# Shamir-Lab/Faucet

Hardware: AMD Instinct MI355X
Metric: canonical k-mers/s (load+scan) at k=31, 100bp reads; % HBM roofline (higher is better)
Workload: dtype u64

## Files before the change

### faucet_amd/_lib.py

```python
from __future__ import annotations

import ctypes as C
import os

HERE = os.path.dirname(os.path.abspath(__file__))
LIB_PATH = os.path.join(HERE, "libfaucet_gpu.so")

OK, ERR_ARG, ERR_HIP, ERR_STATE, ERR_CAPACITY, ERR_NOMEM = range(6)
BLOO1, BLOO2 = 0, 1
FLAG_PROFILE = 1
FLAG_EAGER_FLAGS = 2
FLAG_NO_RESIDENT = 4
FLAG_RECORD_STOPS = 8
FLAG_MERCY = 16
FLAG_KEY_ORDER_FROM_START = 32
STOP_POS_MASK, STOP_FORWARD, STOP_FIRST, STOP_FAKE = 0x0FFFFFFF, 1 << 28, 1 << 29, 1 << 30
TABLE_ENTRY_BYTES = 32


class Params(C.Structure):
    _fields_ = [("k", C.c_int32), ("j", C.c_int32), ("max_spacer_dist", C.c_int32), ("n_hash", C.c_int32),
                ("tai", C.c_uint64), ("device", C.c_int32), ("flags", C.c_int32), ("junction_capacity", C.c_uint64),
                ("max_batch_bases", C.c_uint64), ("stream", C.c_void_p), ("walk_window_span", C.c_uint64)]

# ... 105 lines not shown
    "fgpu_probe_bloom_junction": (C.c_int, [_vp, _vp, _u64, _vp]),
    "fgpu_stage3_set_junctions": (C.c_int, [_vp, _vp, _vp, _u64]),
    "fgpu_stage3_find_neighbors": (C.c_int, [_vp, _vp, _vp, _u64, _i32, _vp, _P(_u64), _vp, _u64]),
    "fgpu_stage3_contig_words": (_u64, [_i32, _i32]),
    "fgpu_kernel_times": (C.c_int, [_vp, _P(KernelTime), C.c_int]),
    "fgpu_kernel_times_reset": (C.c_int, [_vp]),
    "fgpu_profile_enable": (C.c_int, [_vp, C.c_int]),
    "fgpu_diag_stream_copy": (C.c_int, [_vp, _u64, C.c_int, _P(_f64)]),
    "fgpu_diag_random_access": (C.c_int, [_vp, _u64, _u64, C.c_int, C.c_int, _P(_f64)]),
    "fgpu_diag_ko_trace": (C.c_int, [_vp, _vp, _u64, _P(_u64)]),
    "fgpu_diag_ko_stamps": (C.c_int, [_vp, _vp, _u64, _P(_u64)]),
    "fgpu_diag_binned_chain": (C.c_int, [_vp, _u64, _u64, _u64, C.c_int, C.c_int, C.c_int, _P(_f64), _P(_f64), _P(_f64), _P(_f64), _P(_f64), _P(C.c_int)]),
    "fgpu_diag_device_attr": (C.c_int, [_vp, _P(_i32), _P(_i32), _P(_i32), _P(_i32)]),
    "fgpu_diag_walk_probe": (C.c_int, [_vp, _P(_u64)]),
    "fgpu_diag_load_split": (C.c_int, [_vp, _P(_u64), _P(_u64)]),
    "fgpu_diag_scan_replays": (C.c_int, [_vp, _P(_u64)]),
    "fgpu_diag_host_waits": (C.c_int, [_vp, _P(_u64), _P(_f64)]),
    "fgpu_diag_load_tables": (C.c_int, [_vp, _u64, _P(_f64), _P(_f64), _P(_f64)]),
    "fgpu_diag_pair_placements": (C.c_int, [_vp, C.c_int, _u64, _P(_f64)]),
    "fgpu_diag_late_flags": (C.c_int, [_vp, _P(_u64)]),
    "fgpu_diag_binned_probes": (C.c_int, [_vp, _u64, _u64, _u64, C.c_int, _P(_f64), _P(_f64), _P(_f64), _P(_f64)]),
    "fgpu_scan_pairs_devptr": (C.c_int, [_vp, C.c_int, _P(_vp), _P(_u64)]),
    "fgpu_device_alloc": (C.c_int, [_vp, _u64, _P(_vp)]),
    "fgpu_device_free": (C.c_int, [_vp, _vp]),
    "fgpu_device_copy": (C.c_int, [_vp, _vp, _vp, _u64]),
    "fgpu_device_zero": (C.c_int, [_vp, _vp, _u64]),
    "fgpu_group_create": (C.c_int, [C.c_int, C.c_int, _P(_vp)]),
    "fgpu_group_destroy": (None, [_vp]),
    "fgpu_group_attach": (C.c_int, [_vp, C.c_int, _vp]),
    "fgpu_group_abort": (None, [_vp]),
# ... 39 lines not shown
```

### faucet_amd/api.py

```python
from __future__ import annotations

import ctypes as C

import numpy as np

from . import _lib as L


class FaucetGpuError(RuntimeError):
    pass


def _check(rc, ctx=None):
    if rc != L.OK:
        msg = L.load().fgpu_last_error(ctx).decode(errors="replace") if ctx is not None else L.load().fgpu_last_error(None).decode()
        raise FaucetGpuError(f"libfaucet_gpu error {rc}: {msg}")


def solve_p1(estimated_kmers: int, singletons: int, fp: float = 0.04) -> float:
    it = C.c_int32(0)
    p1 = L.load().fgpu_solve_p1(estimated_kmers, singletons, C.c_float(fp), C.byref(it))
    if p1 < 0:
        raise ValueError("p1 solver: root not bracketed (singletons must be > 0 and < estimated_kmers)")
    return p1
# ... 458 lines not shown
    def diag_scan_replays(self) -> int:
        n = C.c_uint64(0)
        self._c(self.lib.fgpu_diag_scan_replays(self.h, C.byref(n)))
        return int(n.value)

    def diag_late_flags(self) -> dict:
        out = (C.c_uint64 * 3)()
        self._c(self.lib.fgpu_diag_late_flags(self.h, out))
        return {"noted": int(out[0]), "conflicts": int(out[1]), "swept": int(out[2])}

    def diag_load_split(self) -> dict:
        a, b = C.c_uint64(0), C.c_uint64(0)
        self._c(self.lib.fgpu_diag_load_split(self.h, C.byref(a), C.byref(b)))
        return {"in_mark": int(a.value), "pending": int(b.value)}

    def diag_binned_probes(self, table_bytes: int, n_probes: int, slice_bytes: int = 4 << 20, iters: int = 3) -> dict:
        v = [C.c_double(0) for _ in range(4)]
        self._c(self.lib.fgpu_diag_binned_probes(self.h, table_bytes, n_probes, slice_bytes, iters, *[C.byref(x) for x in v]))
        return dict(zip(("direct_per_s", "binned_per_s", "bin_ms", "probe_ms"), [float(x.value) for x in v]))

    def diag_binned_chain(self, table_bytes: int, n_items: int, slice_bytes: int = 4 << 20, n_hash: int = 3, fill_byte: int = 0x29, iters: int = 3) -> dict:
        v = [C.c_double(0) for _ in range(5)]
        eq = C.c_int(0)
        self._c(self.lib.fgpu_diag_binned_chain(self.h, table_bytes, n_items, slice_bytes, n_hash, fill_byte, iters, *[C.byref(x) for x in v], C.byref(eq)))
        d = dict(zip(("direct_ms", "bin_ms", "first_ms", "rest_ms", "survivors_share"), [float(x.value) for x in v]))
        d["equal"] = bool(eq.value)
        return d

    def diag_ko_trace(self) -> np.ndarray:
        out = np.zeros((1 << 21, 4), dtype=np.uint64)
# ... 116 lines not shown
```

### faucet_amd/csrc/api.hip

```cpp
#include <cstdio>
#include <algorithm>
#include <string>

#include <chrono>
#include <thread>

#include "fgpu_ctx.h"

int fgpu_scan_export_impl(fgpu_ctx* ctx, void* dev_entries, uint64_t cap_entries, uint64_t* d_stamps, uint64_t* n_entries);
int fgpu_scan_import_impl(fgpu_ctx* ctx, const void* dev_entries, uint64_t n);
int fgpu_scan_download_impl(fgpu_ctx* ctx, uint64_t* keys_host, fgpu_junction* recs_host, uint64_t cap, uint64_t* n_out);

static thread_local std::string g_create_error;

int g_fgpu_trace = getenv("FGPU_TRACE") && getenv("FGPU_TRACE")[0] == '1';

int fgpu_ensure(fgpu_ctx* ctx, DevBuf* b, uint64_t bytes) {
    if (b->bytes >= bytes && b->p) return FGPU_OK;
    if (b->p) {
        FGPU_HIP(fgpu_sync_stream(ctx, ctx->stream));
        FGPU_HIP(hipFree(b->p));
        b->p = nullptr;
        b->bytes = 0;
    } else {
// ... 134 lines not shown
static bool is_pow2(uint64_t x) { return x && !(x & (x - 1)); }

static void journal_recycle(fgpu_ctx* ctx);
static int journal_add(fgpu_ctx* ctx, BatchBufs* b, const fgpu_reads* reads);
static int scan_replay(fgpu_ctx* ctx);

int fgpu_check_reads(fgpu_ctx* ctx, const fgpu_reads* r) {
    if (!r || (r->n_reads && (!r->bases || !r->offsets))) { ctx->err = "null read batch"; return FGPU_ERR_ARG; }
    return FGPU_OK;
}

void fgpu_load_pass_policy(fgpu_ctx* ctx) {
    static const char* carry_env = getenv("FGPU_CARRY_MODE");
    ctx->carry_by_set = carry_env ? carry_env[0] == 's' && carry_env[1] == 'e' : ctx->prm.tai == (1ULL << 31);
    ctx->epoch_positions = ctx->swept_positions = 0;
    ctx->sweep_num = ctx->sweep_den = 1;
    const char* sweep_env = getenv("FGPU_SWEEP_RATIO");
    if (sweep_env) {
        unsigned n = 1, d = 1;
        if (sscanf(sweep_env, "%u/%u", &n, &d) == 2 && d > 0) { ctx->sweep_num = n; ctx->sweep_den = d; }
    }
    {
        const char* e = getenv("FGPU_SWEEP_MIN_FRAC");
        const double frac = e ? atof(e) : 16.0;
        ctx->sweep_min = frac > 0.0 ? (uint64_t)((double)ctx->prm.tai / frac / (double)std::max(1, ctx->prm.n_hash)) : 0;
    }
}
int fgpu_load_pass_counters(fgpu_ctx* ctx) {
    FGPU_HIP(hipMemsetAsync(ctx->counters, 0, sizeof(DevCounters), ctx->stream));
    memset(&ctx->load_stats, 0, sizeof(ctx->load_stats));
// ... 193 lines not shown
    void* ptrs[] = {ctx->lp.bits, ctx->lp.first, ctx->short_pf, ctx->bloo1, ctx->bloo2, ctx->first, ctx->pair, ctx->rec, ctx->slice_first, ctx->slice_pair, ctx->jkeys, ctx->jrecs, ctx->jstamps, ctx->jfilter, ctx->wkeys,
                    ctx->wbits, ctx->uf_parent, ctx->cl_count, ctx->cl_offset, ctx->cl_fill, ctx->cl_fail, ctx->ko_hk, ctx->ko_occ, ctx->ko_piece, ctx->cl_members, ctx->cl_roots, ctx->counters,
                    ctx->wdesc};
    for (void* p : ptrs) if (p) hipFree(p);
    stop_queue_recycle(ctx);
    for (StopBatch& f : ctx->stop_pool) hipHostFree(f.data);
    ctx->stop_pool.clear();
    if (ctx->counters_host) hipHostFree(ctx->counters_host);
    if (ctx->fb_host) hipHostFree(ctx->fb_host);
    if (ctx->wstream) { hipStreamSynchronize(ctx->wstream); hipStreamDestroy(ctx->wstream); }
    if (ctx->cstream) { hipStreamSynchronize(ctx->cstream); hipStreamDestroy(ctx->cstream); }
    if (ctx->ostream) { hipStreamSynchronize(ctx->ostream); hipStreamDestroy(ctx->ostream); }
    if (ctx->ev_walked) hipEventDestroy(ctx->ev_walked);
    if (ctx->ev_listed) hipEventDestroy(ctx->ev_listed);
    if (ctx->ev_settled) hipEventDestroy(ctx->ev_settled);
    for (int q = 0; q < 2; q++) if (ctx->ev_uf_reset[q]) hipEventDestroy(ctx->ev_uf_reset[q]);
    if (ctx->own_stream && ctx->stream) hipStreamDestroy(ctx->stream);
    for (ResidentBatch* r : ctx->resident) delete r;
    for (PackedBlock* b : ctx->packed) delete b;
    for (JournalBatch* j : ctx->journal) delete j;
    for (JournalBatch* j : ctx->journal_pool) delete j;
    for (BatchBufs* b : ctx->all_batches) {
        if (b->pure_done) hipEventDestroy(b->pure_done);
        if (b->walk_done) hipEventDestroy(b->walk_done);
        delete b;
    }
    delete ctx;
}

int fgpu_synchronize(fgpu_ctx* ctx) {
// ... 29 lines not shown
        if (e != hipSuccess) {
            ctx->err = std::string("hipMalloc of the interleaved filter pair failed: ") + hipGetErrorString(e);
            ctx->pair = nullptr;
            return FGPU_ERR_NOMEM;
        }
        if (int rc = fgpu_place_pair(ctx)) return rc;
    }
    ctx->shard_times = (keep_carry & FGPU_LOAD_SHARD_TIMES) != 0;
    ctx->shard_planes = (keep_carry & FGPU_LOAD_SHARD_PLANES) != 0 && !ctx->shard_times && ctx->prm.n_hash <= 4;
    ctx->fixup_ready = false;
    ctx->scan_resident_base = 0;
    ctx->pass_positions = ctx->pass_batches = 0;
    ctx->pass_empty_carry = !(keep_carry & FGPU_LOAD_KEEP_CARRY);
    keep_carry &= FGPU_LOAD_KEEP_CARRY;
    fgpu_load_pass_policy(ctx);
    if (!ctx->rec_layout) FGPU_HIP(hipMemsetAsync(ctx->first, 0xFF, ctx->prm.tai * 4, ctx->stream));
    fgpu_resident_reset(ctx, true);
    if (!keep_carry) FGPU_HIP(hipMemsetAsync(ctx->bloo1, 0, ctx->bloom_bytes, ctx->stream));
    FGPU_HIP(hipMemsetAsync(ctx->bloo2, 0, ctx->bloom_bytes, ctx->stream));
    int rc = fgpu_load_pair_begin(ctx);
    if (rc) return rc;
    if ((rc = fgpu_load_pass_counters(ctx))) return rc;
    ctx->phase = 1;
    return FGPU_OK;
}

int fgpu_load_batch(fgpu_ctx* ctx, const fgpu_reads* reads) {
    if (!ctx) return FGPU_ERR_ARG;
    if (ctx->phase != 1) { ctx->err = "load_batch outside load_begin/load_end"; return FGPU_ERR_STATE; }
    int rc = fgpu_check_reads(ctx, reads);
// ... 875 lines not shown
    FGPU_HIP(hipMemcpy(&cnt, (const char*)ctx->ko_trace.p + 8, 8, hipMemcpyDeviceToHost));
    if (cnt > 4096) cnt = 4096;
    if (cnt * 1024 > cap_words) cnt = cap_words / 1024;
    if (cnt && out) FGPU_HIP(hipMemcpy(out, (const char*)ctx->ko_trace.p + (8ULL << 23), cnt * 1024 * 8, hipMemcpyDeviceToHost));
    *n_pieces = cnt;
    return FGPU_OK;
}

int fgpu_diag_load_split(fgpu_ctx* ctx, uint64_t* in_mark, uint64_t* pending) {
    if (!ctx || !in_mark || !pending) return FGPU_ERR_ARG;
    *in_mark = ctx->load_mark_hits;
    *pending = ctx->load_mark_pending;
    return FGPU_OK;
}

int fgpu_diag_ovw(fgpu_ctx* ctx, uint64_t out[6]) {
    if (!ctx || !out) return FGPU_ERR_ARG;
    for (int i = 0; i < 4; i++) out[i] = ctx->counters_host->ovw[i];
    out[4] = ctx->counters_host->ovw_kept;
    out[5] = ctx->counters_host->ko_overflows;
    return FGPU_OK;
}

int fgpu_diag_prepared_refresh(fgpu_ctx* ctx, uint64_t out[4]) {
    if (!ctx || !out) return FGPU_ERR_ARG;
    out[0] = ctx->refresh_full;
    out[1] = ctx->refresh_delta;
    out[2] = ctx->delta_keys;
    out[3] = ctx->refresh_mismatch;
    return FGPU_OK;
// ... 46 lines not shown
```

### faucet_amd/csrc/fgpu_ctx.h

```cpp
#pragma once
#include <chrono>
#include <hip/hip_runtime.h>
#include <stdint.h>
#include <stdio.h>
#include <string.h>

#include <string>
#include <thread>
#include <vector>

#include "../../include/faucet_gpu.h"
#include <deque>

#include "fgpu_device.h"

#define FGPU_PADW 8
#define FGPU_USUAL_SPAN (1ULL << 26)
#define FGPU_MAX_SPAN (1ULL << 26)

struct DevBuf {
    void*    p = nullptr;
    uint64_t bytes = 0;
};

struct BatchBufs {
    DevBuf codes, bad;
    DevBuf readflag;
    DevBuf pending;
    DevBuf sure;
    DevBuf fail;
    DevBuf same;
    DevBuf valid, pm, ps, ff, fb, cf0, cf1, cb0, cb1, inF, inB;
    DevBuf lk;
    DevBuf cand;
    uint32_t cand_gen = 0;
    DevBuf nF, nB, need;
    DevBuf kh;
    DevBuf cr;
    DevBuf ps_prefix;
    DevBuf pieces;
    DevBuf sF, sB;
    DevBuf piece_read;
    DevBuf stop_off, stop_out;
    const uint64_t* d_offs = nullptr;
    uint64_t seq = 0;
    bool stops_pending = false;
// ... 141 lines not shown
    int bg_rc = 0;
    std::string bg_err;

    uint32_t* bloo1 = nullptr;
    uint64_t epoch_positions = 0;
    uint64_t swept_positions = 0;
    bool shard_times = false;
    bool shard_planes = false;
    bool fixup_ready = false;
    uint64_t pass_positions = 0;
    uint32_t cur_tb = 0;
    bool pass_empty_carry = true;
    uint64_t pass_batches = 0;
    uint64_t sweep_min = 0;
    uint32_t sweep_num = 1, sweep_den = 1;
    bool carry_by_set = false;
    uint32_t* bloo2 = nullptr;
    uint32_t* first = nullptr;
    uint2* pair = nullptr;
    uint32_t* rec = nullptr;
    bool rec_layout = false;
    uint64_t bloom_bytes = 0;
    int phase = 0;
    uint64_t slice_lo = 0, slice_n = 0;
    uint32_t* slice_first = nullptr;
    uint2* slice_pair = nullptr;
    uint64_t slice_first_bytes = 0, slice_pair_bytes = 0;
    bool slice_committed = false;
    bool slice_mercy = false;
    bool slice_probe_owed = false;
// ... 283 lines not shown
```

### faucet_amd/csrc/load.hip

```cpp
#include <algorithm>

#include "fgpu_ctx.h"
#include "fgpu_flags.h"
#include "load_common.h"

namespace {

template <int REC>
__global__ void __launch_bounds__(256) k_load_mark(const uint64_t* __restrict__ codes, const uint64_t* __restrict__ bad,
                                                   uint64_t T, uint64_t n_words, FdParams fp, Filt<REC> f, uint32_t tb,
                                                   uint64_t* __restrict__ pending, uint64_t plane_stride, uint64_t* __restrict__ sure, DevCounters* cnt) {
    unsigned long long n_ok = 0, n_hit = 0, n_pend = 0;
    const uint64_t total = n_words * 64;
    for (uint64_t p = (uint64_t)blockIdx.x * blockDim.x + threadIdx.x; p < total; p += (uint64_t)gridDim.x * blockDim.x) {
        bool ok = p < T && fd_window_ok(bad, p, fp.k);
        bool pend = false, hit = false;
        uint32_t miss_bits = 0;
        if (ok) {
            n_ok++;
            uint64_t canon = fd_canon(fd_kmer_at(codes, p, fp.k), fp.k);
            uint64_t hA, hB;
            fd_hash_pair(canon, fp.tai_mask, hA, hB);
            uint32_t missing = 0, b2_missing = 0;
            uint64_t h = hA;
// ... 263 lines not shown
        const int g = fd_lane() & 15;
        uint32_t lo = g < 8 ? nib << (4 * g) : 0u, hi = g >= 8 ? nib << (4 * (g - 8)) : 0u;
#pragma unroll
        for (int o = 1; o < 16; o <<= 1) {
            lo |= __shfl_xor(lo, o, 64);
            hi |= __shfl_xor(hi, o, 64);
        }
        if (g == 0) {
            const uint64_t w = i >> 3;
            if (lo) pair[w].x |= lo;
            if (hi) pair[w + 1].x |= hi;
        }
    }
}

template <int REC>
__global__ void __launch_bounds__(256) k_carry_set(const uint64_t* __restrict__ codes, const uint64_t* __restrict__ bad, uint64_t T,
                                                   uint64_t n_words, FdParams fp, Filt<REC> f, const uint64_t* __restrict__ sure) {
    const uint64_t total = n_words * 64;
    for (uint64_t p = (uint64_t)blockIdx.x * blockDim.x + threadIdx.x; p < total; p += (uint64_t)gridDim.x * blockDim.x) {
        if (!(p < T && fd_window_ok(bad, p, fp.k)) || ((sure[p >> 6] >> (p & 63)) & 1ULL)) continue;
        uint64_t hA, hB;
        fd_hash_pair(fd_canon(fd_kmer_at(codes, p, fp.k), fp.k), fp.tai_mask, hA, hB);
        uint64_t h = hA;
        for (int i = 0; i < fp.n_hash; i++) {
            const uint32_t bit = 1u << (h & 31);
            if (!(f.word(h)[0] & bit)) atomicOr(f.word(h), bit);
            h = (h + hB) & fp.tai_mask;
        }
    }
// ... 160 lines not shown
        ctx->resident_open = false;
        return FGPU_OK;
    }
    r->T = bb.T;
    r->n_words = bb.n_words;
    r->tb = ctx->cur_tb;
    FGPU_HIP(hipMemcpyAsync(r->codes.p, bb.codes.p, parts[0], hipMemcpyDeviceToDevice, ctx->stream));
    FGPU_HIP(hipMemcpyAsync(r->bad.p, bb.bad.p, pb, hipMemcpyDeviceToDevice, ctx->stream));
    FGPU_HIP(hipMemcpyAsync(r->sure.p, bb.sure.p, pb, hipMemcpyDeviceToDevice, ctx->stream));
    if (parts[3]) FGPU_HIP(hipMemcpyAsync(r->fail.p, bb.fail.p, parts[3], hipMemcpyDeviceToDevice, ctx->stream));
    ctx->resident_count++;
    ctx->resident_bytes += kept;
    return FGPU_OK;
}

int fgpu_load_sweep(fgpu_ctx* ctx) {
    if (ctx->epoch_positions == 0) return FGPU_OK;
    if (ctx->phase == 3) {
        if (ctx->slice_n) FGPU_LAUNCH("slice_carry_update", k_carry_from_first, 4096, 256, ctx->slice_pair, (const uint4*)ctx->slice_first, ctx->slice_n);
    } else if (ctx->rec_layout) {
        FGPU_LAUNCH("carry_update", k_carry_from_rec, 8192, 256, ctx->rec, ctx->prm.tai / 32);
    } else {
        FGPU_LAUNCH("carry_update", k_carry_from_first, 4096, 256, ctx->pair, (const uint4*)ctx->first, ctx->prm.tai);
    }
    ctx->swept_positions += ctx->epoch_positions;
    ctx->epoch_positions = 0;
    return FGPU_OK;
}

int fgpu_epoch_before_batch(fgpu_ctx* ctx, uint64_t span) {
    if (!ctx->carry_by_set && !ctx->shard_times && ctx->epoch_positions + span >= 0xFFFFFFF0ULL) return fgpu_load_sweep(ctx);
    return FGPU_OK;
}
int fgpu_epoch_after_batch(fgpu_ctx* ctx, uint64_t span) {
    if (ctx->carry_by_set) return FGPU_OK;
    ctx->epoch_positions += span;
    if (ctx->epoch_positions * ctx->sweep_den >= ctx->swept_positions * ctx->sweep_num && ctx->epoch_positions >= ctx->sweep_min) return fgpu_load_sweep(ctx);
    return FGPU_OK;
}

template <int REC>
static int load_batch(fgpu_ctx* ctx, const Filt<REC>& f, uint32_t tb, bool keep_fail) {
    BatchBufs& bb = *ctx->cur;
    const uint64_t plane_stride = bb.n_words + FGPU_PADW;
    const unsigned grid = fgpu_grid(bb.n_words * 64, 256);
    static const int resolve_sm = getenv("FGPU_RESOLVE_SM") ? atoi(getenv("FGPU_RESOLVE_SM")) : 4096;
    FGPU_LAUNCH("load_mark", k_load_mark<REC>, grid, 256, (const uint64_t*)bb.codes.p, (const uint64_t*)bb.bad.p, bb.T, bb.n_words, ctx->fd, f,
                tb, (uint64_t*)bb.pending.p, plane_stride, (uint64_t*)bb.sure.p, ctx->counters);
    if (ctx->fd.n_hash <= MISS_PLANES && resolve_sm && !keep_fail) {
        const unsigned rgrid = (unsigned)std::min<uint64_t>((bb.n_words + 255) / 256, (uint64_t)std::max(resolve_sm, 64));
        FGPU_LAUNCH("load_resolve", k_load_resolve_sm<REC>, rgrid, 256, (const uint64_t*)bb.codes.p, bb.n_words, ctx->fd, f, tb,
                    (const uint64_t*)bb.pending.p, plane_stride, (unsigned long long*)bb.sure.p, ctx->counters);
// ... 19 lines not shown

int fgpu_stage_load(fgpu_ctx* ctx) {
    BatchBufs& bb = *ctx->cur;
    if (bb.T == 0) return FGPU_OK;
    const uint64_t plane_stride = bb.n_words + FGPU_PADW;
    int rc = fgpu_ensure_b(ctx, &bb.pending, (MISS_PLANES + 1) * plane_stride * 8);
    if (rc) return rc;
    if ((rc = fgpu_ensure_b(ctx, &bb.sure, (bb.n_words + FGPU_PADW) * 8))) return rc;
    if ((rc = fgpu_util_count_segments(ctx, bb.bad.p, bb.n_words, ctx->fd.k))) return rc;
    const uint64_t span = bb.n_words * 64;
    if ((rc = fgpu_epoch_before_batch(ctx, span))) return rc;
    if (ctx->shard_times && ctx->pass_positions + span >= 0xFFFFFFF0ULL) {
        ctx->err = "FGPU_LOAD_SHARD_TIMES: the pass exceeds 2^32 stream positions (FGPU_LOAD_SHARD_PLANES has no such limit)";
        return FGPU_ERR_CAPACITY;
    }
    const uint32_t tb = ctx->shard_times ? (uint32_t)ctx->pass_positions : ctx->carry_by_set ? 0u : (uint32_t)ctx->epoch_positions;
    const bool keep_fail = ctx->shard_planes && ctx->fd.n_hash <= MISS_PLANES;
    if (keep_fail && (rc = fgpu_ensure_b(ctx, &bb.fail, MISS_PLANES * plane_stride * 8))) return rc;
    ctx->cur_tb = tb;
    ctx->pass_positions += span;
    if ((rc = with_layout(ctx, [&](auto f) { return load_batch(ctx, f, tb, keep_fail); }))) return rc;
    if ((rc = fgpu_epoch_after_batch(ctx, span))) return rc;
    return fgpu_resident_keep(ctx);
}

int fgpu_load_pair_begin(fgpu_ctx* ctx) {
    if (ctx->rec_layout) FGPU_LAUNCH("pair_join", k_rec_init, 8192, 256, ctx->rec, (const uint32_t*)ctx->bloo1, ctx->bloom_bytes / 4);
    else FGPU_LAUNCH("pair_join", k_pair_join, 2048, 256, ctx->pair, (const uint32_t*)ctx->bloo1, (const uint32_t*)nullptr, ctx->bloom_bytes / 4);
    return FGPU_OK;
}
int fgpu_load_pair_end(fgpu_ctx* ctx) {
    if (ctx->phase == 3) {
        FGPU_HIP(hipMemsetAsync(ctx->bloo1, 0, ctx->bloom_bytes, ctx->stream));
        FGPU_HIP(hipMemsetAsync(ctx->bloo2, 0, ctx->bloom_bytes, ctx->stream));
        if (ctx->slice_n)
            FGPU_LAUNCH("pair_split", k_pair_split, 2048, 256, (const uint2*)ctx->slice_pair, ctx->bloo1 + ctx->slice_lo / 32,
                        ctx->bloo2 + ctx->slice_lo / 32, ctx->slice_n / 32);
    } else if (ctx->rec_layout) {
        FGPU_LAUNCH("pair_split", k_rec_split, 4096, 256, (const uint32_t*)ctx->rec, ctx->bloo1, ctx->bloo2, ctx->bloom_bytes / 4);
    } else {
        FGPU_LAUNCH("pair_split", k_pair_split, 2048, 256, (const uint2*)ctx->pair, ctx->bloo1, ctx->bloo2, ctx->bloom_bytes / 4);
    }
    return FGPU_OK;
}

int fgpu_stage_fixup(fgpu_ctx* ctx, const uint32_t* prefix) {
// ... 55 lines not shown
```

### faucet_amd/csrc/scan_pure.hip

```cpp
#include <algorithm>

#include "fgpu_ctx.h"
#include "fgpu_flags.h"

namespace {

__global__ void __launch_bounds__(256) k_scan_same(const uint64_t* __restrict__ codes, const uint64_t* __restrict__ kept_codes, uint64_t n_code_words,
                                                   const uint64_t* __restrict__ bad, const uint64_t* __restrict__ kept_bad, uint64_t n_words,
                                                   uint32_t* same) {
    bool differ = false;
    for (uint64_t i = (uint64_t)blockIdx.x * blockDim.x + threadIdx.x; i < n_code_words; i += (uint64_t)gridDim.x * blockDim.x) {
        differ |= codes[i] != kept_codes[i];
        if (i < n_words) differ |= bad[i] != kept_bad[i];
    }
    if (__ballot(differ) && fd_lane() == 0) *same = 0;
}

__global__ void __launch_bounds__(256) k_scan_valid(const uint64_t* __restrict__ codes, const uint64_t* __restrict__ bad,
                                                    uint64_t T, uint64_t n_words, FdParams fp, const uint32_t* __restrict__ bloom,
                                                    const uint64_t* __restrict__ sure, const uint32_t* __restrict__ same,
                                                    uint64_t* __restrict__ valid, DevCounters* cnt) {
    unsigned long long n_ok = 0, n_reused = 0;
    const uint64_t total = n_words * 64;
    const bool reuse = sure && *same != 0;
// ... 419 lines not shown
        for (int nt = 0; nt < 4; nt++) {
            const uint64_t e = ((km << 2) | (uint64_t)nt) & fp.kmask;
            if (fd_bloom_contains_canon(bloom, fd_canon(e, fp.k), fp.tai_mask, fp.n_hash) && jcheck_dfs(e, fp, bloom)) {
                if (r != -1) { r = -2; break; }
                r = nt;
            }
        }
    } else {
        int paths = 0;
        for (int nt = 0; nt < 4; nt++) paths += jcheck_dfs(((km << 2) | (uint64_t)nt) & fp.kmask, fp, bloom) ? 1 : 0;
        r = paths > 1 ? 1 : 0;
    }
    out[i] = (signed char)r;
}

}

void fgpu_touch_scan_pure() {
    hipFuncAttributes attr;
    (void)hipFuncGetAttributes(&attr, (const void*)k_scan_same);
}

int fgpu_util_probe_stage3(fgpu_ctx* ctx, const uint64_t* d_kmers, uint64_t n, int mode, signed char* d_out) {
    FGPU_LAUNCH("probe_stage3", k_probe_stage3, fgpu_blocks(n, 256), 256, d_kmers, n, mode, ctx->fd, (const uint32_t*)ctx->bloo2, d_out);
    return FGPU_OK;
}

int fgpu_stage_scan_pure(fgpu_ctx* ctx, uint64_t* n_pieces) {
    BatchBufs& bb = *ctx->cur;
    *n_pieces = 0;
    bb.n_pieces = 0;
    if (bb.T == 0) return FGPU_OK;
    const uint64_t wb = (bb.n_words + FGPU_PADW) * 8;
    int rc;
    DevBuf* planes[] = {&bb.valid, &bb.pm, &bb.ps, &bb.ff, &bb.fb, &bb.cf0, &bb.cf1, &bb.cb0, &bb.cb1, &bb.inF, &bb.inB, &bb.lk, &bb.nF, &bb.nB, &bb.need};
    for (DevBuf* b : planes)
        if ((rc = fgpu_ensure_b(ctx, b, wb))) return rc;
    if ((rc = fgpu_ensure_b(ctx, &bb.ps_prefix, (bb.n_words + FGPU_PADW + bb.n_words / SCAN_BLOCK + 2) * 4))) return rc;
    const double t_a = fgpu_host_now();
    FGPU_HIP(hipMemsetAsync(bb.valid.p, 0, wb, ctx->stream));
    FGPU_HIP(hipMemsetAsync(bb.pm.p, 0, wb, ctx->stream));
    FGPU_HIP(hipMemsetAsync(bb.ps.p, 0, wb, ctx->stream));

    const unsigned grid = fgpu_grid(bb.n_words * 64, 256);
    const unsigned wgrid = fgpu_grid(bb.n_words, 256);
    if ((rc = fgpu_util_count_segments(ctx, ctx->cur->bad.p, ctx->cur->n_words, ctx->fd.k + 2 * ctx->fd.j + 1))) return rc;
    const uint64_t kept_index = ctx->scan_resident_base + ctx->scan_batch_index;
    const ResidentBatch* kept = kept_index < ctx->resident_count ? ctx->resident[kept_index] : nullptr;
    ctx->scan_batch_index++;
    if (kept && (kept->T != bb.T || kept->n_words != bb.n_words)) kept = nullptr;
    if (kept) {
        if ((rc = fgpu_ensure_b(ctx, &bb.same, 64))) return rc;
        FGPU_HIP(hipMemsetAsync(bb.same.p, 0x01, 4, ctx->stream));
        const uint64_t ncw = 2 * bb.n_words;
        FGPU_LAUNCH("scan_same", k_scan_same, fgpu_grid(ncw, 256), 256, (const uint64_t*)bb.codes.p, (const uint64_t*)kept->codes_p(), ncw,
                    (const uint64_t*)bb.bad.p, (const uint64_t*)kept->bad_p(), bb.n_words, (uint32_t*)bb.same.p);
    }
// ... 19 lines not shown
    bb.max_piece_span = ctx->counters_host->max_read_len + 64;
    const uint64_t np = ctx->counters_host->pieces - ctx->scan_pieces_seen;
    ctx->scan_pieces_seen = ctx->counters_host->pieces;
    *n_pieces = np;
    bb.n_pieces = np;
    if ((rc = fgpu_ensure_b(ctx, &bb.pieces, (np + 1) * sizeof(uint2)))) return rc;
    if (np) {
        FGPU_LAUNCH("piece_list", k_scan_piece_list, wgrid, 256, (const uint64_t*)bb.ps.p, (const uint64_t*)bb.pm.p,
                    (const uint32_t*)prefix, bb.n_words, (uint2*)bb.pieces.p);
        if (ctx->record_stops) {
            if ((rc = fgpu_ensure_b(ctx, &bb.piece_read, np * 4))) return rc;
            FGPU_LAUNCH("piece_read", k_scan_piece_read, fgpu_blocks(np, 256), 256, (const uint2*)bb.pieces.p, np, bb.d_offs, bb.n_reads,
                        (uint32_t*)bb.piece_read.p);
        }
        if ((rc = fgpu_stage_scan_need(ctx))) return rc;
        DevBuf* outs[] = {&bb.ff, &bb.fb, &bb.cf0, &bb.cf1, &bb.cb0, &bb.cb1};
        for (DevBuf* o : outs) FGPU_HIP(hipMemsetAsync(o->p, 0, wb, ctx->stream));
        const unsigned flags_grid = (unsigned)std::min<uint64_t>(std::max<uint64_t>(bb.n_words / 16, 1), 2 * FGPU_GRID_BLOCKS);
        static const int sm_blocks = getenv("FGPU_FLAGS_SM_BLOCKS") ? atoi(getenv("FGPU_FLAGS_SM_BLOCKS")) : 4096;
        if (ctx->fd.j <= 1 && sm_blocks > 0) {
            const unsigned sm_grid = (unsigned)std::min<uint64_t>(std::max<uint64_t>((bb.n_words + 255) / 256, 1), (uint64_t)sm_blocks);
            static const int sm_slots = getenv("FGPU_FLAGS_SM_SLOTS") ? atoi(getenv("FGPU_FLAGS_SM_SLOTS")) : 1;
#define FGPU_FLAGS_SM(SLOTS)                                                                                                        \
    FGPU_LAUNCH("scan_flags", k_scan_flags_sm<SLOTS>, sm_grid, 256, (const uint64_t*)bb.codes.p, (const uint64_t*)bb.pm.p,           \
                (const uint64_t*)bb.need.p, bb.T, bb.n_words, ctx->fd, (const uint32_t*)ctx->bloo2, (unsigned long long*)bb.ff.p,    \
                (unsigned long long*)bb.fb.p, (unsigned long long*)bb.cf0.p, (unsigned long long*)bb.cf1.p,                         \
                (unsigned long long*)bb.cb0.p, (unsigned long long*)bb.cb1.p, ctx->counters)
            if (sm_slots <= 1) FGPU_FLAGS_SM(1);
            else if (sm_slots == 2) FGPU_FLAGS_SM(2);
            else if (sm_slots == 3) FGPU_FLAGS_SM(3);
            else FGPU_FLAGS_SM(4);
#undef FGPU_FLAGS_SM
// ... 11 lines not shown
```

### faucet_amd/csrc/scan_walk.hip

```cpp
#include <cstring>
#include <algorithm>

#include "fgpu_flags.h"
#include "walk_tables.h"

namespace {

__device__ __forceinline__ uint32_t uf_find(uint32_t* parent, uint32_t x) {
    uint32_t p = ld_agent(&parent[x]);
    while (p != x) {
        uint32_t gp = ld_agent(&parent[p]);
        if (gp != p) atomicMin(&parent[x], gp);
        x = p;
        p = gp;
    }
    return x;
}

__device__ __forceinline__ void uf_union(uint32_t* parent, uint32_t a, uint32_t b) {
    for (;;) {
        a = uf_find(parent, a);
        b = uf_find(parent, b);
        if (a == b) return;
        if (a < b) { uint32_t t = a; a = b; b = t; }
// ... 2258 lines not shown
    FGPU_LAUNCH("iota", k_iota_u32, 64, 256, ctx->uf_parent, (uint64_t)ctx->wmax);
    FGPU_LAUNCH("iota", k_iota_u32, 64, 256, ctx->uf_parent + ctx->wmax, (uint64_t)ctx->wmax);
    FGPU_HIP(hipMemsetAsync(ctx->cl_count, 0, 2 * ctx->wmax * 4, ctx->stream));
    FGPU_HIP(hipMemsetAsync(ctx->cl_offset, 0xFF, 2 * ctx->wmax * 4, ctx->stream));
    FGPU_HIP(hipMemsetAsync(ctx->cl_fail, 0, 2 * ctx->wmax * 4, ctx->stream));
    FGPU_HIP(hipMemsetAsync(ctx->ko_hk, 0xFF, (size_t)ctx->ko_hk_cap * 4 * 2, ctx->stream));
    FGPU_HIP(hipMemsetAsync(ctx->ko_hk + 2 * (size_t)ctx->ko_hk_cap, 0, (size_t)ctx->ko_hk_cap * 4, ctx->stream));
    FGPU_HIP(hipMemsetAsync(ctx->ko_piece, 0, (size_t)ctx->wmax * 4 * 2 + 64, ctx->stream));
    return FGPU_OK;
}

int fgpu_stage_scan_need(fgpu_ctx* ctx) {
    BatchBufs& bb = *ctx->cur;
    const uint64_t wb = (bb.n_words + FGPU_PADW) * 8;
    const bool eager = (ctx->prm.flags & FGPU_FLAG_EAGER_FLAGS) || ctx->eager_runtime || ctx->eager_scan;
    FGPU_HIP(hipMemsetAsync(bb.need.p, eager ? 0xFF : 0, wb, ctx->stream));
    if (!bb.n_pieces) return FGPU_OK;
    if (int rc = fgpu_ensure_b(ctx, &bb.kh, (bb.n_words + FGPU_PADW) * 64 * 4)) return rc;

    static const int need_tight = getenv("FGPU_NEED_TIGHT") ? atoi(getenv("FGPU_NEED_TIGHT")) : 2;
    JTable jt = make_jt(ctx);
    FGPU_LAUNCH("need_lookup", k_need_lookup, fgpu_grid(bb.n_words * 64, 256), 256, (const uint64_t*)bb.codes.p, (const uint64_t*)bb.pm.p,
                bb.n_words, ctx->fd, jt, (uint64_t*)bb.nF.p, (uint64_t*)bb.nB.p, (uint32_t*)bb.kh.p, (uint64_t)0);
    if (eager) return FGPU_OK;
    FGPU_LAUNCH("need_prewalk", k_need_prewalk, fgpu_grid(bb.n_pieces, 256), 256, (const uint64_t*)bb.codes.p, (const uint2*)bb.pieces.p,
                bb.n_pieces, ctx->fd, jt, (const uint64_t*)bb.nF.p, (const uint64_t*)bb.nB.p, (unsigned long long*)bb.need.p, need_tight);
    return FGPU_OK;
}

int fgpu_scan_refresh_planes(fgpu_ctx* ctx, BatchBufs* b) {
    if (!b->n_pieces || !b->T) return FGPU_OK;
// ... 409 lines not shown
    }
    *span_now = span;
    return FGPU_OK;
}

int fgpu_stage_scan_walk(fgpu_ctx* ctx, uint64_t n_pieces) {
    if (!n_pieces) return FGPU_OK;
    const WalkKnobs& kn = walk_knobs();
    BatchBufs& bb = *ctx->cur;
    int rc;
    const uint64_t wbytes = (bb.n_words + FGPU_PADW) * 8;
    Planes pl{(const uint64_t*)bb.codes.p, (const uint64_t*)bb.pm.p, (const uint64_t*)bb.ps.p, (const uint32_t*)bb.ps_prefix.p,
              (const uint64_t*)bb.ff.p, (const uint64_t*)bb.fb.p, (const uint64_t*)bb.cf0.p, (const uint64_t*)bb.cf1.p,
              (const uint64_t*)bb.cb0.p, (const uint64_t*)bb.cb1.p, (uint64_t*)bb.nF.p, (uint64_t*)bb.nB.p, (const uint2*)bb.pieces.p,
              (uint64_t*)bb.lk.p, (const uint64_t*)bb.need.p, nullptr, nullptr, (const uint32_t*)bb.kh.p, nullptr};
    if ((rc = fgpu_ensure_b(ctx, &bb.cr, wbytes))) return rc;
    pl.cr = (unsigned long long*)bb.cr.p;
    if (ctx->record_stops) {
        if ((rc = fgpu_ensure_b(ctx, &bb.sF, wbytes)) || (rc = fgpu_ensure_b(ctx, &bb.sB, wbytes))) return rc;
        pl.sF = (unsigned long long*)bb.sF.p;
        pl.sB = (unsigned long long*)bb.sB.p;
    }
    const uint64_t span = ctx->window_span;
    const uint64_t ext = bb.max_piece_span;
    if (ctx->max_span + ext + 64 > ctx->wcap) {
        ctx->err = "a read of " + std::to_string(ext) + " bases is longer than the walk's window tables allow";
        return FGPU_ERR_CAPACITY;
    }
    if (ext >= (1ULL << (STAMP_SHIFT - 1)) - 64) {
        ctx->err = "a read of " + std::to_string(ext) + " bases is longer than the junction creation stamps allow (2^19 windows)";
        return FGPU_ERR_CAPACITY;
    }
    hipStream_t walk_stream = kn.no_overlap ? ctx->stream : ctx->wstream;
    hipStream_t ovw_stream = (kn.ovw_beside && !kn.no_overlap && ctx->ostream) ? ctx->ostream : walk_stream;
    WalkBatch wb{bb, pl, make_jt(ctx), bb.T, ext, ctx->scan_piece_base, walk_stream, ovw_stream, false, &ctx->delta_ring[ctx->delta_next % FGPU_DELTA_RING]};
    const uint64_t T = wb.T;
    ctx->launch_stream = walk_stream;
    if (bb.pure_done) FGPU_HIP(hipStreamWaitEvent(walk_stream, bb.pure_done, 0));
    if (ctx->dbg_stall_us) FGPU_LAUNCH("debug_stall", k_debug_stall, 1, 1, (unsigned long long)ctx->dbg_stall_us * 100ULL);
    if (ctx->refresh_snapshot && (rc = walk_refresh_prepared(ctx, bb, wb.jt, walk_stream, &wb.cand_ok))) return rc;
    if (ctx->record_stops) {
        FGPU_HIP(hipMemsetAsync(bb.sF.p, 0, wbytes, walk_stream));
        FGPU_HIP(hipMemsetAsync(bb.sB.p, 0, wbytes, walk_stream));
    }
    FGPU_HIP(hipMemsetAsync(bb.cr.p, 0, wbytes, walk_stream));
    {
        const uint64_t now = ctx->counters_host->n_junctions;
        ctx->delta_hist[ctx->delta_next % FGPU_DELTA_RING] = now;
        const uint64_t back = ctx->delta_next >= (uint64_t)(FGPU_DELTA_RING - 1) ? ctx->delta_hist[(ctx->delta_next - (FGPU_DELTA_RING - 1)) % FGPU_DELTA_RING] : 0;
        ctx->delta_ring_keys = now > back ? now - back : 0;
        ctx->delta_batch_base = now;
    }
    if ((rc = fgpu_ensure_b(ctx, &wb.created->list, (bb.n_words + FGPU_PADW) * 64 * 4)) || (rc = fgpu_ensure(ctx, &wb.created->count, 64))) return rc;
    FGPU_HIP(hipMemsetAsync(wb.created->count.p, 0, 8, walk_stream));
    const int stage_tok = fgpu_prof_begin(ctx, "walk_stage");
    ctx->prof_suppress = !ctx->prof_walk_detail;
    uint64_t span_now = span;
    const bool whole_batch = wb.cand_ok && !kn.no_whole_batch && !ctx->prm.walk_window_span && ctx->calib_left <= 0 && span * 2 >= T && span < T && T <= ctx->max_span &&
                             bb.n_pieces <= ctx->wmax;
    for (uint64_t lo = 0, step = 0; lo < T; lo += step) {
// ... 31 lines not shown
```

### include/faucet_gpu.h

```cpp
#ifndef FAUCET_GPU_H
#define FAUCET_GPU_H

#include <stdint.h>

#ifdef __cplusplus
extern "C" {
#endif

#define FGPU_ABI_VERSION 3

enum {
    FGPU_OK = 0,
    FGPU_ERR_ARG = 1,
    FGPU_ERR_HIP = 2,
    FGPU_ERR_STATE = 3,
    FGPU_ERR_CAPACITY = 4,
    FGPU_ERR_NOMEM = 5
};

enum { FGPU_BLOO1 = 0, FGPU_BLOO2 = 1 };

typedef struct fgpu_ctx fgpu_ctx;

typedef struct {
// ... 220 lines not shown
int fgpu_diag_ko_trace(fgpu_ctx* ctx, uint64_t* out, uint64_t cap_records, uint64_t* n);
int fgpu_diag_ko_stamps(fgpu_ctx* ctx, uint64_t* out, uint64_t cap_words, uint64_t* n_pieces);
int fgpu_diag_random_access(fgpu_ctx* ctx, uint64_t table_bytes, uint64_t n_access, int mode, int iters, double* access_per_s);
int fgpu_diag_load_tables(fgpu_ctx* ctx, uint64_t n_access, double* pair_loads_per_s, double* first_atomics_per_s, double* mixed_items_per_s);
int fgpu_diag_pair_placements(fgpu_ctx* ctx, int k, uint64_t n_items, double* items_per_s);
int fgpu_diag_binned_probes(fgpu_ctx* ctx, uint64_t table_bytes, uint64_t n_probes, uint64_t slice_bytes, int iters, double* direct_per_s,
                            double* binned_per_s, double* bin_ms, double* probe_ms);
int fgpu_diag_walk_probe(fgpu_ctx* ctx, uint64_t out[4]);
int fgpu_diag_scan_replays(fgpu_ctx* ctx, uint64_t* replays);
int fgpu_diag_host_waits(fgpu_ctx* ctx, uint64_t* waits, double* ms);
int fgpu_diag_late_flags(fgpu_ctx* ctx, uint64_t out[3]);
int fgpu_diag_long_pairs(fgpu_ctx* ctx, uint64_t out[6]);
int fgpu_diag_ovw(fgpu_ctx* ctx, uint64_t out[6]);
int fgpu_diag_ovw_tables(fgpu_ctx* ctx, uint64_t* high_water, uint64_t* capacity);
int fgpu_diag_load_split(fgpu_ctx* ctx, uint64_t* in_mark, uint64_t* pending);
int fgpu_diag_device_attr(fgpu_ctx* ctx, int32_t* mem_clock_khz, int32_t* mem_bus_bits, int32_t* l2_bytes, int32_t* compute_units);

#ifdef __cplusplus
}
#endif
#endif
```

Measured before the change: 5.943 billion.

## Overlap carry sweeps on a side stream and batch-clear scan planes in one kernel

```diff
diff --git a/faucet_amd/_lib.py b/faucet_amd/_lib.py
--- a/faucet_amd/_lib.py
+++ b/faucet_amd/_lib.py
@@ -143,6 +143,7 @@
     "fgpu_diag_device_attr": (C.c_int, [_vp, _P(_i32), _P(_i32), _P(_i32), _P(_i32)]),
     "fgpu_diag_walk_probe": (C.c_int, [_vp, _P(_u64)]),
     "fgpu_diag_load_split": (C.c_int, [_vp, _P(_u64), _P(_u64)]),
+    "fgpu_diag_load_sweeps": (C.c_int, [_vp, _P(_u64), _P(_u64)]),
     "fgpu_diag_scan_replays": (C.c_int, [_vp, _P(_u64)]),
     "fgpu_diag_host_waits": (C.c_int, [_vp, _P(_u64), _P(_f64)]),
     "fgpu_diag_load_tables": (C.c_int, [_vp, _u64, _P(_f64), _P(_f64), _P(_f64)]),
diff --git a/faucet_amd/api.py b/faucet_amd/api.py
--- a/faucet_amd/api.py
+++ b/faucet_amd/api.py
@@ -496,6 +496,11 @@
         self._c(self.lib.fgpu_diag_load_split(self.h, C.byref(a), C.byref(b)))
         return {"in_mark": int(a.value), "pending": int(b.value)}
 
+    def diag_load_sweeps(self) -> dict:
+        a, b = C.c_uint64(0), C.c_uint64(0)
+        self._c(self.lib.fgpu_diag_load_sweeps(self.h, C.byref(a), C.byref(b)))
+        return {"serial": int(a.value), "beside": int(b.value)}
+
     def diag_binned_probes(self, table_bytes: int, n_probes: int, slice_bytes: int = 4 << 20, iters: int = 3) -> dict:
         v = [C.c_double(0) for _ in range(4)]
         self._c(self.lib.fgpu_diag_binned_probes(self.h, table_bytes, n_probes, slice_bytes, iters, *[C.byref(x) for x in v]))
diff --git a/faucet_amd/csrc/api.hip b/faucet_amd/csrc/api.hip
--- a/faucet_amd/csrc/api.hip
+++ b/faucet_amd/csrc/api.hip
@@ -172,6 +172,9 @@
     static const char* carry_env = getenv("FGPU_CARRY_MODE");
     ctx->carry_by_set = carry_env ? carry_env[0] == 's' && carry_env[1] == 'e' : ctx->prm.tai == (1ULL << 31);
     ctx->epoch_positions = ctx->swept_positions = 0;
+    ctx->clock_positions = 0;
+    ctx->sweeps_serial = ctx->sweeps_beside = 0;
+    ctx->sweep_overlap = false;
     ctx->sweep_num = ctx->sweep_den = 1;
     const char* sweep_env = getenv("FGPU_SWEEP_RATIO");
     if (sweep_env) {
@@ -395,6 +398,8 @@
     if (ctx->ev_walked) hipEventDestroy(ctx->ev_walked);
     if (ctx->ev_listed) hipEventDestroy(ctx->ev_listed);
     if (ctx->ev_settled) hipEventDestroy(ctx->ev_settled);
+    if (ctx->ev_epoch_end) hipEventDestroy(ctx->ev_epoch_end);
+    if (ctx->ev_sweep_done) hipEventDestroy(ctx->ev_sweep_done);
     for (int q = 0; q < 2; q++) if (ctx->ev_uf_reset[q]) hipEventDestroy(ctx->ev_uf_reset[q]);
     if (ctx->own_stream && ctx->stream) hipStreamDestroy(ctx->stream);
     for (ResidentBatch* r : ctx->resident) delete r;
@@ -454,6 +459,14 @@
     ctx->pass_empty_carry = !(keep_carry & FGPU_LOAD_KEEP_CARRY);
     keep_carry &= FGPU_LOAD_KEEP_CARRY;
     fgpu_load_pass_policy(ctx);
+    {
+        const char* e = getenv("FGPU_SWEEP_OVERLAP");
+        ctx->sweep_overlap = e && e[0] == '1' && !ctx->rec_layout && !ctx->carry_by_set && !ctx->shard_times && !ctx->shard_planes &&
+                             !(ctx->prm.flags & FGPU_FLAG_MERCY);
+        const char* w = getenv("FGPU_DEBUG_CLOCK_WRAP");
+        const unsigned long long wrap = w ? strtoull(w, nullptr, 10) : 0;
+        ctx->clock_wrap = wrap > 0 && wrap < 0xFFFFFFF0ULL ? wrap : 0xFFFFFFF0ULL;
+    }
     if (!ctx->rec_layout) FGPU_HIP(hipMemsetAsync(ctx->first, 0xFF, ctx->prm.tai * 4, ctx->stream));
     fgpu_resident_reset(ctx, true);
     if (!keep_carry) FGPU_HIP(hipMemsetAsync(ctx->bloo1, 0, ctx->bloom_bytes, ctx->stream));
@@ -1359,6 +1372,13 @@
     return FGPU_OK;
 }
 
+int fgpu_diag_load_sweeps(fgpu_ctx* ctx, uint64_t* serial, uint64_t* beside) {
+    if (!ctx || !serial || !beside) return FGPU_ERR_ARG;
+    *serial = ctx->sweeps_serial;
+    *beside = ctx->sweeps_beside;
+    return FGPU_OK;
+}
+
 int fgpu_diag_ovw(fgpu_ctx* ctx, uint64_t out[6]) {
     if (!ctx || !out) return FGPU_ERR_ARG;
     for (int i = 0; i < 4; i++) out[i] = ctx->counters_host->ovw[i];
diff --git a/faucet_amd/csrc/fgpu_ctx.h b/faucet_amd/csrc/fgpu_ctx.h
--- a/faucet_amd/csrc/fgpu_ctx.h
+++ b/faucet_amd/csrc/fgpu_ctx.h
@@ -30,6 +30,7 @@
     DevBuf sure;
     DevBuf fail;
     DevBuf same;
+    DevBuf zeroed;
     DevBuf valid, pm, ps, ff, fb, cf0, cf1, cb0, cb1, inF, inB;
     DevBuf lk;
     DevBuf cand;
@@ -201,6 +202,12 @@
     uint64_t pass_batches = 0;
     uint64_t sweep_min = 0;
     uint32_t sweep_num = 1, sweep_den = 1;
+    bool sweep_overlap = false;
+    uint64_t clock_positions = 0;
+    uint64_t clock_wrap = 0xFFFFFFF0ULL;
+    bool sweep_in_flight = false;
+    hipEvent_t ev_epoch_end = nullptr, ev_sweep_done = nullptr;
+    uint64_t sweeps_serial = 0, sweeps_beside = 0;
     bool carry_by_set = false;
     uint32_t* bloo2 = nullptr;
     uint32_t* first = nullptr;
diff --git a/faucet_amd/csrc/load.hip b/faucet_amd/csrc/load.hip
--- a/faucet_amd/csrc/load.hip
+++ b/faucet_amd/csrc/load.hip
@@ -301,6 +301,28 @@
     }
 }
 
+__global__ void __launch_bounds__(256) k_carry_before(uint2* pair, const uint4* __restrict__ first4, uint64_t tai, uint32_t t0) {
+    const uint64_t n4 = tai / 4;
+    for (uint64_t i = (uint64_t)blockIdx.x * blockDim.x + threadIdx.x; i < n4; i += (uint64_t)gridDim.x * blockDim.x) {
+        const uint4 v = first4[i];
+        const uint32_t nib = (v.x < t0 ? 1u : 0u) | (v.y < t0 ? 2u : 0u) | (v.z < t0 ? 4u : 0u) | (v.w < t0 ? 8u : 0u);
+        const int g = fd_lane() & 15;
+        uint32_t lo = g < 8 ? nib << (4 * g) : 0u, hi = g >= 8 ? nib << (4 * (g - 8)) : 0u;
+#pragma unroll
+        for (int o = 1; o < 16; o <<= 1) {
+            lo |= __shfl_xor(lo, o, 64);
+            hi |= __shfl_xor(hi, o, 64);
+        }
+        if (g == 0) {
+            const uint64_t w = i >> 3;
+            uint32_t* const c0 = &pair[w].x;
+            uint32_t* const c1 = &pair[w + 1].x;
+            if (lo & ~*c0) atomicOr(c0, lo);
+            if (hi & ~*c1) atomicOr(c1, hi);
+        }
+    }
+}
+
 template <int REC>
 __global__ void __launch_bounds__(256) k_carry_set(const uint64_t* __restrict__ codes, const uint64_t* __restrict__ bad, uint64_t T,
                                                    uint64_t n_words, FdParams fp, Filt<REC> f, const uint64_t* __restrict__ sure) {
@@ -491,8 +513,17 @@
     return FGPU_OK;
 }
 
+static int sweep_join(fgpu_ctx* ctx) {
+    if (!ctx->sweep_in_flight) return FGPU_OK;
+    FGPU_HIP(hipStreamWaitEvent(ctx->stream, ctx->ev_sweep_done, 0));
+    ctx->sweep_in_flight = false;
+    return FGPU_OK;
+}
 int fgpu_load_sweep(fgpu_ctx* ctx) {
+    if (int rc = sweep_join(ctx)) return rc;
+    ctx->clock_positions = 0;
     if (ctx->epoch_positions == 0) return FGPU_OK;
+    ctx->sweeps_serial++;
     if (ctx->phase == 3) {
         if (ctx->slice_n) FGPU_LAUNCH("slice_carry_update", k_carry_from_first, 4096, 256, ctx->slice_pair, (const uint4*)ctx->slice_first, ctx->slice_n);
     } else if (ctx->rec_layout) {
@@ -506,13 +537,39 @@
 }
 
 int fgpu_epoch_before_batch(fgpu_ctx* ctx, uint64_t span) {
+    if (ctx->sweep_overlap) return ctx->clock_positions + span >= ctx->clock_wrap ? fgpu_load_sweep(ctx) : FGPU_OK;
     if (!ctx->carry_by_set && !ctx->shard_times && ctx->epoch_positions + span >= 0xFFFFFFF0ULL) return fgpu_load_sweep(ctx);
     return FGPU_OK;
 }
+
+static int fgpu_load_sweep_beside(fgpu_ctx* ctx) {
+    if (!ctx->cstream) {
+        if (int rc = fgpu_bg_join(ctx)) return rc;
+        if (!ctx->cstream) { ctx->sweep_overlap = false; return fgpu_load_sweep(ctx); }
+    }
+    if (!ctx->ev_epoch_end) {
+        FGPU_HIP(hipEventCreateWithFlags(&ctx->ev_epoch_end, hipEventDisableTiming));
+        FGPU_HIP(hipEventCreateWithFlags(&ctx->ev_sweep_done, hipEventDisableTiming));
+    }
+    FGPU_HIP(hipEventRecord(ctx->ev_epoch_end, ctx->stream));
+    FGPU_HIP(hipStreamWaitEvent(ctx->cstream, ctx->ev_epoch_end, 0));
+    ctx->launch_stream = ctx->cstream;
+    FGPU_LAUNCH("carry_update", k_carry_before, 4096, 256, ctx->pair, (const uint4*)ctx->first, ctx->prm.tai, (uint32_t)ctx->clock_positions);
+    ctx->launch_stream = ctx->stream;
+    FGPU_HIP(hipEventRecord(ctx->ev_sweep_done, ctx->cstream));
+    ctx->sweep_in_flight = true;
+    ctx->sweeps_beside++;
+    ctx->swept_positions += ctx->epoch_positions;
+    ctx->epoch_positions = 0;
+    return FGPU_OK;
+}
+
 int fgpu_epoch_after_batch(fgpu_ctx* ctx, uint64_t span) {
     if (ctx->carry_by_set) return FGPU_OK;
     ctx->epoch_positions += span;
-    if (ctx->epoch_positions * ctx->sweep_den >= ctx->swept_positions * ctx->sweep_num && ctx->epoch_positions >= ctx->sweep_min) return fgpu_load_sweep(ctx);
+    ctx->clock_positions += span;
+    if (ctx->epoch_positions * ctx->sweep_den >= ctx->swept_positions * ctx->sweep_num && ctx->epoch_positions >= ctx->sweep_min)
+        return ctx->sweep_overlap ? fgpu_load_sweep_beside(ctx) : fgpu_load_sweep(ctx);
     return FGPU_OK;
 }
 
@@ -562,14 +619,15 @@
         ctx->err = "FGPU_LOAD_SHARD_TIMES: the pass exceeds 2^32 stream positions (FGPU_LOAD_SHARD_PLANES has no such limit)";
         return FGPU_ERR_CAPACITY;
     }
-    const uint32_t tb = ctx->shard_times ? (uint32_t)ctx->pass_positions : ctx->carry_by_set ? 0u : (uint32_t)ctx->epoch_positions;
+    const uint32_t tb = ctx->shard_times ? (uint32_t)ctx->pass_positions : ctx->carry_by_set ? 0u :
+                        ctx->sweep_overlap ? (uint32_t)ctx->clock_positions : (uint32_t)ctx->epoch_positions;
     const bool keep_fail = ctx->shard_planes && ctx->fd.n_hash <= MISS_PLANES;
     if (keep_fail && (rc = fgpu_ensure_b(ctx, &bb.fail, MISS_PLANES * plane_stride * 8))) return rc;
     ctx->cur_tb = tb;
     ctx->pass_positions += span;
     if ((rc = with_layout(ctx, [&](auto f) { return load_batch(ctx, f, tb, keep_fail); }))) return rc;
-    if ((rc = fgpu_epoch_after_batch(ctx, span))) return rc;
-    return fgpu_resident_keep(ctx);
+    if ((rc = fgpu_resident_keep(ctx))) return rc;
+    return fgpu_epoch_after_batch(ctx, span);
 }
 
 int fgpu_load_pair_begin(fgpu_ctx* ctx) {
@@ -578,6 +636,7 @@
     return FGPU_OK;
 }
 int fgpu_load_pair_end(fgpu_ctx* ctx) {
+    if (int rc = sweep_join(ctx)) return rc;
     if (ctx->phase == 3) {
         FGPU_HIP(hipMemsetAsync(ctx->bloo1, 0, ctx->bloom_bytes, ctx->stream));
         FGPU_HIP(hipMemsetAsync(ctx->bloo2, 0, ctx->bloom_bytes, ctx->stream));
diff --git a/faucet_amd/csrc/scan_pure.hip b/faucet_amd/csrc/scan_pure.hip
--- a/faucet_amd/csrc/scan_pure.hip
+++ b/faucet_amd/csrc/scan_pure.hip
@@ -457,6 +457,10 @@
     out[i] = (signed char)r;
 }
 
+__global__ void __launch_bounds__(256) k_clear16(uint4* __restrict__ p, uint64_t n16) {
+    for (uint64_t i = (uint64_t)blockIdx.x * blockDim.x + threadIdx.x; i < n16; i += (uint64_t)gridDim.x * blockDim.x) p[i] = make_uint4(0u, 0u, 0u, 0u);
+}
+
 }
 
 void fgpu_touch_scan_pure() {
@@ -476,14 +480,20 @@
     if (bb.T == 0) return FGPU_OK;
     const uint64_t wb = (bb.n_words + FGPU_PADW) * 8;
     int rc;
-    DevBuf* planes[] = {&bb.valid, &bb.pm, &bb.ps, &bb.ff, &bb.fb, &bb.cf0, &bb.cf1, &bb.cb0, &bb.cb1, &bb.inF, &bb.inB, &bb.lk, &bb.nF, &bb.nB, &bb.need};
+    DevBuf* planes[] = {&bb.inF, &bb.inB, &bb.lk, &bb.nF, &bb.nB};
     for (DevBuf* b : planes)
         if ((rc = fgpu_ensure_b(ctx, b, wb))) return rc;
     if ((rc = fgpu_ensure_b(ctx, &bb.ps_prefix, (bb.n_words + FGPU_PADW + bb.n_words / SCAN_BLOCK + 2) * 4))) return rc;
+    const bool eager = (ctx->prm.flags & FGPU_FLAG_EAGER_FLAGS) || ctx->eager_runtime || ctx->eager_scan;
+    DevBuf* zeroed[] = {&bb.need, &bb.valid, &bb.pm, &bb.ps, &bb.ff, &bb.fb, &bb.cf0, &bb.cf1, &bb.cb0, &bb.cb1, &bb.cr, &bb.sF, &bb.sB};
+    const uint64_t n_zeroed = ctx->record_stops ? 13 : 11, zstride = (wb + 255) & ~255ULL;
+    if ((rc = fgpu_ensure_b(ctx, &bb.zeroed, n_zeroed * zstride))) return rc;
+    for (uint64_t i = 0; i < 13; i++) *zeroed[i] = i < n_zeroed ? DevBuf{(char*)bb.zeroed.p + i * zstride, wb} : DevBuf{};
     const double t_a = fgpu_host_now();
-    FGPU_HIP(hipMemsetAsync(bb.valid.p, 0, wb, ctx->stream));
-    FGPU_HIP(hipMemsetAsync(bb.pm.p, 0, wb, ctx->stream));
-    FGPU_HIP(hipMemsetAsync(bb.ps.p, 0, wb, ctx->stream));
+    {
+        const uint64_t skip = eager ? zstride : 0, n16 = (n_zeroed * zstride - skip) / 16;
+        FGPU_LAUNCH("clear_planes", k_clear16, fgpu_grid(n16, 256), 256, (uint4*)((char*)bb.zeroed.p + skip), n16);
+    }
 
     const unsigned grid = fgpu_grid(bb.n_words * 64, 256);
     const unsigned wgrid = fgpu_grid(bb.n_words, 256);
@@ -533,8 +543,6 @@
                         (uint32_t*)bb.piece_read.p);
         }
         if ((rc = fgpu_stage_scan_need(ctx))) return rc;
-        DevBuf* outs[] = {&bb.ff, &bb.fb, &bb.cf0, &bb.cf1, &bb.cb0, &bb.cb1};
-        for (DevBuf* o : outs) FGPU_HIP(hipMemsetAsync(o->p, 0, wb, ctx->stream));
         const unsigned flags_grid = (unsigned)std::min<uint64_t>(std::max<uint64_t>(bb.n_words / 16, 1), 2 * FGPU_GRID_BLOCKS);
         static const int sm_blocks = getenv("FGPU_FLAGS_SM_BLOCKS") ? atoi(getenv("FGPU_FLAGS_SM_BLOCKS")) : 4096;
         if (ctx->fd.j <= 1 && sm_blocks > 0) {
diff --git a/faucet_amd/csrc/scan_walk.hip b/faucet_amd/csrc/scan_walk.hip
--- a/faucet_amd/csrc/scan_walk.hip
+++ b/faucet_amd/csrc/scan_walk.hip
@@ -2296,7 +2296,7 @@
     BatchBufs& bb = *ctx->cur;
     const uint64_t wb = (bb.n_words + FGPU_PADW) * 8;
     const bool eager = (ctx->prm.flags & FGPU_FLAG_EAGER_FLAGS) || ctx->eager_runtime || ctx->eager_scan;
-    FGPU_HIP(hipMemsetAsync(bb.need.p, eager ? 0xFF : 0, wb, ctx->stream));
+    if (eager) FGPU_HIP(hipMemsetAsync(bb.need.p, 0xFF, wb, ctx->stream));
     if (!bb.n_pieces) return FGPU_OK;
     if (int rc = fgpu_ensure_b(ctx, &bb.kh, (bb.n_words + FGPU_PADW) * 64 * 4)) return rc;
 
@@ -2736,10 +2736,12 @@
               (const uint64_t*)bb.ff.p, (const uint64_t*)bb.fb.p, (const uint64_t*)bb.cf0.p, (const uint64_t*)bb.cf1.p,
               (const uint64_t*)bb.cb0.p, (const uint64_t*)bb.cb1.p, (uint64_t*)bb.nF.p, (uint64_t*)bb.nB.p, (const uint2*)bb.pieces.p,
               (uint64_t*)bb.lk.p, (const uint64_t*)bb.need.p, nullptr, nullptr, (const uint32_t*)bb.kh.p, nullptr};
-    if ((rc = fgpu_ensure_b(ctx, &bb.cr, wbytes))) return rc;
+    if (!bb.cr.p || bb.cr.bytes < wbytes || (ctx->record_stops && (!bb.sF.p || !bb.sB.p))) {
+        ctx->err = "walk stage: the batch's planes were not made by the pure stage";
+        return FGPU_ERR_STATE;
+    }
     pl.cr = (unsigned long long*)bb.cr.p;
     if (ctx->record_stops) {
-        if ((rc = fgpu_ensure_b(ctx, &bb.sF, wbytes)) || (rc = fgpu_ensure_b(ctx, &bb.sB, wbytes))) return rc;
         pl.sF = (unsigned long long*)bb.sF.p;
         pl.sB = (unsigned long long*)bb.sB.p;
     }
@@ -2761,11 +2763,6 @@
     if (bb.pure_done) FGPU_HIP(hipStreamWaitEvent(walk_stream, bb.pure_done, 0));
     if (ctx->dbg_stall_us) FGPU_LAUNCH("debug_stall", k_debug_stall, 1, 1, (unsigned long long)ctx->dbg_stall_us * 100ULL);
     if (ctx->refresh_snapshot && (rc = walk_refresh_prepared(ctx, bb, wb.jt, walk_stream, &wb.cand_ok))) return rc;
-    if (ctx->record_stops) {
-        FGPU_HIP(hipMemsetAsync(bb.sF.p, 0, wbytes, walk_stream));
-        FGPU_HIP(hipMemsetAsync(bb.sB.p, 0, wbytes, walk_stream));
-    }
-    FGPU_HIP(hipMemsetAsync(bb.cr.p, 0, wbytes, walk_stream));
     {
         const uint64_t now = ctx->counters_host->n_junctions;
         ctx->delta_hist[ctx->delta_next % FGPU_DELTA_RING] = now;
diff --git a/include/faucet_gpu.h b/include/faucet_gpu.h
--- a/include/faucet_gpu.h
+++ b/include/faucet_gpu.h
@@ -258,6 +258,7 @@
 int fgpu_diag_ovw(fgpu_ctx* ctx, uint64_t out[6]);
 int fgpu_diag_ovw_tables(fgpu_ctx* ctx, uint64_t* high_water, uint64_t* capacity);
 int fgpu_diag_load_split(fgpu_ctx* ctx, uint64_t* in_mark, uint64_t* pending);
+int fgpu_diag_load_sweeps(fgpu_ctx* ctx, uint64_t* serial, uint64_t* beside);
 int fgpu_diag_device_attr(fgpu_ctx* ctx, int32_t* mem_clock_khz, int32_t* mem_bus_bits, int32_t* l2_bytes, int32_t* compute_units);
 
 #ifdef __cplusplus
```

Measured after the change: 5.874 billion. 1.2% lower.
